# IRVLUTD/GraspTrajOpt

Hardware: AMD Instinct MI355X
Metric: grasp trajectories/sec (higher is better)
Workload: dtype f64

## Files before the change

grasptrajopt_amd/csrc/gto_api.hip:

```cpp
#include <hip/hip_runtime.h>
#include <hipcub/hipcub.hpp>

#include <algorithm>
#include <atomic>
#include <climits>
#include <cmath>
#include <cstdio>
#include <cstdlib>
#include <cstring>
#include <string>
#include <chrono>
#include <memory>
#include <mutex>
#include <thread>
#include <utility>
#include <vector>

#include <sys/prctl.h>

#include "gto_kernels.h"

#define GTO_VERSION GTO_ABI_VERSION
#ifndef GTO_OBS_DEEP_PD
#define GTO_OBS_DEEP_PD 8
// ... 92 lines not shown
  void* p = nullptr;
  size_t cap = 0;
};

struct gto_handle {
  int device = 0;
  hipStream_t stream = nullptr;
  bool own_stream = true;
  std::string err;
  gto_solver_opts opts;
  RobotDev rb;
  RobotDev* d_rb = nullptr;
  double *d_px = nullptr, *d_py = nullptr, *d_pz = nullptr;
  int32_t *d_plink = nullptr, *d_perm = nullptr;
  Chunk* d_chunks = nullptr;
  PbChunk* d_pbchunks = nullptr;
  int pb_C = 0;
  std::vector<SceneDev> scenes;
  SceneDev* d_scenes = nullptr;
  size_t d_scenes_cap = 0;
  DevBuf state, Qcur, Qtry, vis, screw, blocks, goalblk, ssfixed, ndone, qf, livebuf, qfs, wrecbuf, itembuf;
  DevBuf counters;
  unsigned long long last_counters[4] = {0, 0, 0, 0};
  int32_t* h_ndone = nullptr;
  unsigned long long* h_progress = nullptr;
  unsigned long long* d_progress = nullptr;
  unsigned progress_tag = 0;
  Tunables tu;
  int spec_kmax = 1;
  long long* dbg = nullptr;
  std::vector<std::pair<void*, size_t>> spare;
  DevBuf in[8], out[8];
// ... 207 lines not shown
  rb.frame_free_mask = 0u;
  for (int i = 0; i < d->n_frames; ++i)
    if (rb.opt_of_frame[i] < 0) rb.frame_free_mask |= 1u << i;
  for (int i = 0; i < d->n_frames; ++i) {
    const int p = rb.parent[i];
    if (p >= 0 && p != i - 1 && rb.xst_slot[p] < 0) rb.xst_slot[p] = rb.n_xst++;
  }
  {
    for (int i = 0; i < d->n_frames; ++i) {
      const int p = rb.parent[i], l = rb.link_of_frame[i];
      const int src = p < 0 ? 0 : (p == i - 1 ? 1 : 2 + rb.xst_slot[p]);
      const bool moving_link = l >= 0 && (rb.frame_anc[rb.link_frame[l]] != 0u);
      rb.pb_ctl[i] = (src & 7) | (((rb.xst_slot[i] + 1) & 7) << 4) | ((moving_link ? 1 : 0) << 8);
      rb.pb_par[i] = -1;
      if (rb.joint_type[i] != GTO_JOINT_FIXED && rb.opt_of_frame[i] < 0) rb.pb_par[i] = rb.pb_npar, rb.pb_parf[rb.pb_npar++] = i;
    }
    double D = 0.0, maxp = 0.0;
    for (int i = 0; i < d->n_frames; ++i) {
      const double* ox = d->origin_xyz + 3 * i;
      D += std::sqrt(ox[0] * ox[0] + ox[1] * ox[1] + ox[2] * ox[2]);
      if (rb.joint_type[i] == GTO_JOINT_PRISMATIC) {
        const int j = rb.opt_of_frame[i];
        D += j >= 0 ? std::max(std::fabs(rb.lower[j]), std::fabs(rb.upper[j])) : 2.0;
      }
    }
    for (int l = 0; l < d->n_links; ++l) {
      const double* vx = d->visual_xyz + 3 * l;
      maxp = std::max(maxp, std::sqrt(vx[0] * vx[0] + vx[1] * vx[1] + vx[2] * vx[2]));
    }
    double maxr = 0.0;
// ... 256 lines not shown
    while (spec_kmax < GTO_KSPEC && lm_lds_bytes(opts->T, spec_kmax + 1) <= 160 * 1024 - 256) ++spec_kmax;

  int ndev = 0;
  if (hipGetDeviceCount(&ndev) != hipSuccess || ndev == 0)
    return fail(nullptr, GTO_ERR_NO_DEVICE, "no HIP device visible: the GTO solve path has no CPU fallback");
  if (device >= ndev) return fail(nullptr, GTO_ERR_INVALID_ARG, "device index out of range");
  if (device >= 0 && hipSetDevice(device) != hipSuccess) return fail(nullptr, GTO_ERR_HIP, "hipSetDevice failed");

  gto_handle* h = new gto_handle();
  if (device >= 0) h->device = device;
  else (void)hipGetDevice(&h->device);
  h->opts = *opts;
  h->tu = tu;
  std::memcpy(&h->rb, &rb, sizeof rb);
  h->pb_C = t->pb_C;
  h->np = np;
  h->lm_lds = lm_lds;
  h->spec_kmax = spec_kmax;
  if (tu.debug_timing) { (void)hipMalloc((void**)&h->dbg, 256 * sizeof(long long)); (void)hipMemset(h->dbg, 0, 256 * sizeof(long long)); }
  auto up = [&](void** dst, const void* src, size_t bytes) -> bool {
    if (hipMalloc(dst, bytes) != hipSuccess) return false;
    return hipMemcpy(*dst, src, bytes, hipMemcpyHostToDevice) == hipSuccess;
  };
  const size_t P = t->px.size();
  if (hipStreamCreateWithFlags(&h->stream, hipStreamNonBlocking) != hipSuccess) { gto_destroy(h); return fail(nullptr, GTO_ERR_HIP, "hipStreamCreate failed"); }
  const bool ok = up((void**)&h->d_rb, &h->rb, sizeof h->rb) && up((void**)&h->d_px, t->px.data(), P * sizeof(double)) &&
                  up((void**)&h->d_py, t->py.data(), P * sizeof(double)) && up((void**)&h->d_pz, t->pz.data(), P * sizeof(double)) &&
                  up((void**)&h->d_plink, t->plink.data(), P * sizeof(int32_t)) && up((void**)&h->d_perm, t->perm.data(), P * sizeof(int32_t)) &&
                  up((void**)&h->d_chunks, t->chunks.data(), t->chunks.size() * sizeof(Chunk)) &&
                  up((void**)&h->d_pbchunks, t->pbchunks.data(), t->pbchunks.size() * sizeof(PbChunk));
  if (!ok) { gto_destroy(h); return fail(nullptr, GTO_ERR_ALLOC, "device allocation failed in gto_create"); }
  const size_t lds = std::min<size_t>((size_t)lay.total_doubles * sizeof(double), 160 * 1024);
  hipError_t e = hipSuccess;
  for (int v = 0; v < 8 && e == hipSuccess; ++v) e = raise_dynamic_lds((const void*)obstacle_kernel(np, v & 1, v & 2, v & 4), lds);
  if (e == hipSuccess) e = wide ? raise_dynamic_lds((const void*)k_lm_step_wide<16>, lm_lds) : raise_dynamic_lds((const void*)k_lm_step<4, 1>, lm_lds);
  if (e == hipSuccess && !wide) e = raise_dynamic_lds((const void*)k_lm_step<8, GTO_KSPEC>, lm_lds_bytes(opts->T, spec_kmax));
  if (e != hipSuccess) { gto_destroy(h); return fail(nullptr, GTO_ERR_HIP, "hipFuncSetAttribute failed"); }
  *out = h;
  return GTO_OK;
}

void gto_destroy(gto_handle* h) {
  if (!h) return;
  (void)hipSetDevice(h->device);
  if (h->stream) (void)hipStreamSynchronize(h->stream);
// ... 3 lines not shown
      (void)hipFree((void*)s.c_all);
      if (s.r_obs != s.r_all) (void)hipFree((void*)s.r_obs);
      (void)hipFree((void*)s.r_all);
      if (s.d_obs != s.d_all) (void)hipFree((void*)s.d_obs);
      (void)hipFree((void*)s.d_all);
    }
  }
  (void)hipFree(h->d_scenes);
  (void)hipFree(h->d_rb);
  (void)hipFree(h->d_px);
  (void)hipFree(h->d_py);
  (void)hipFree(h->d_pz);
  (void)hipFree(h->d_plink);
  (void)hipFree(h->d_perm);
  (void)hipFree(h->d_chunks);
  (void)hipFree(h->d_pbchunks);
  DevBuf* bufs[] = {&h->zws, &h->counters, &h->state, &h->Qcur, &h->Qtry, &h->vis, &h->screw, &h->blocks, &h->goalblk, &h->ssfixed, &h->ndone, &h->qf, &h->livebuf, &h->qfs, &h->wrecbuf, &h->itembuf};
  if (h->h_ndone) (void)hipHostFree(h->h_ndone);
  if (h->h_progress) (void)hipHostFree(h->h_progress);
  for (DevBuf* b : bufs) (void)hipFree(b->p);
  for (auto& sp_ : h->spare) (void)hipFree(sp_.first);
  for (auto& b : h->in) (void)hipFree(b.p);
  for (auto& b : h->out) (void)hipFree(b.p);
  for (auto& b : h->pin_in) if (b.p) (void)hipHostFree(b.p);
  for (auto& b : h->pin_out) if (b.p) (void)hipHostFree(b.p);
  for (auto e : h->ev) (void)hipEventDestroy(e);
  if (h->stream && h->own_stream) (void)hipStreamDestroy(h->stream);
  for (int l = 0; l < GTO_MAX_LANES; ++l) {
    if (h->lane_stream[l]) (void)hipStreamDestroy(h->lane_stream[l]);
    if (h->lane_event[l]) (void)hipEventDestroy(h->lane_event[l]);
  }
  delete h;
}

int gto_set_opts(gto_handle* h, const gto_solver_opts* o) {
  if (!h || !o) return GTO_ERR_INVALID_ARG;
  std::string why;
  if (!validate_opts(o, why)) return fail(h, GTO_ERR_INVALID_ARG, why);
  if (o->T != h->opts.T) return fail(h, GTO_ERR_INVALID_ARG, "T cannot change after gto_create");
  h->opts = *o;
  return GTO_OK;
}

static int sync_scene_table(gto_handle* h) {
  size_t n = h->scenes.size();
  if (n > h->d_scenes_cap) {
    if (h->d_scenes) HIPCHK(h, hipFree(h->d_scenes));
    h->d_scenes = nullptr;
    size_t cap = std::max<size_t>(16, n * 2);
    HIPCHK(h, hipMalloc((void**)&h->d_scenes, cap * sizeof(SceneDev)));
    h->d_scenes_cap = cap;
  }
  HIPCHK(h, hipMemcpy(h->d_scenes, h->scenes.data(), n * sizeof(SceneDev), hipMemcpyHostToDevice));
  return GTO_OK;
}

static int free_scene(gto_handle* h, SceneDev& s) {
  if (s.valid == 1) {
    if (s.c_obs != s.c_all) HIPCHK(h, hipFree((void*)s.c_obs));
    HIPCHK(h, hipFree((void*)s.c_all));
// ... 611 lines not shown
}

static int enqueue_round(gto_handle* h, const SolveCall& c, LaneCtx& ln, int lane_index, const RoundPlan& p) {
  const int B = c.B, T = c.T;
  SolveParams& lsp = ln.sp;
  lsp.interleave = p.interleave;
  lsp.round = ln.k;
  lsp.parity = ln.k & 1;
  lsp.k_eval = ln.k_prev;
  int rc;
  if ((rc = launch_obstacle(h, ln.st, ln.bp, lsp, B, p.obs))) return rc;
  if (h->profiling && (rc = prof_begin(h, ln.st, p.step == STEP_FEW ? GTO_PROF_STEP_FEW : GTO_PROF_STEP, p.in_flight))) return rc;
  if (p.step == STEP_FEW) {
    lsp.k_acc = p.k_acc, lsp.k_rej = p.k_rej, lsp.spec_streak = p.spec_streak;
    lsp.pb_next = 0, lsp.static_pos = 0;
    hipLaunchKernelGGL((k_lm_step<8, GTO_KSPEC>), dim3(p.span), dim3(512), lm_lds_bytes(T, p.k_next), ln.st, h->d_rb, h->d_pbchunks, ln.bp, lsp, B);
  } else if (p.step == STEP_FULL) {
    lsp.k_acc = lsp.k_rej = 1;
    lsp.pb_next = p.pb_next, lsp.static_pos = p.static_pos;
    hipLaunchKernelGGL((k_lm_step<4, 1>), dim3(p.span), dim3(256), h->lm_lds, ln.st, h->d_rb, h->d_pbchunks, ln.bp, lsp, B);
  } else {
    hipLaunchKernelGGL(k_lm_step_wide<16>, dim3(p.in_flight), dim3(GTO_WIDE_NT), h->lm_lds, ln.st, h->d_rb, ln.bp, lsp, B,
                       (double*)h->zws.p + (size_t)c.lane_zws[lane_index] * (T - 2) * h->np * h->np);
  }
  if (h->profiling && (rc = prof_end(h, ln.st))) return rc;
  ln.span_prev = p.static_pos ? p.span : 0;
  ln.items_ready = p.pb_next;
  ln.k_prev = p.k_next;
  ln.pb_off = p.pb_off;
  ln.ratio_max = p.ratio_max;
  ln.k++;
  return GTO_OK;
}

static void read_progress(unsigned tag, LaneCtx& ln) {
// ... 141 lines not shown
}

static int print_debug_stamps(gto_handle* h, hipStream_t st) {
  HIPCHK(h, hipStreamSynchronize(st));
  long long t[256];
  HIPCHK(h, hipMemcpy(t, h->dbg, sizeof t, hipMemcpyDeviceToHost));
  fprintf(stderr, "[gto dbg] step-kernel phases (cycles) P0+P1 %lld | P2 %lld | diag %lld | dense %lld | back %lld | P4 %lld | P5 %lld | s_dense %lld\n",
          t[1] - t[0], t[2] - t[1], t[3] - t[2], t[4] - t[3], t[5] - t[4], t[6] - t[5], t[7] - t[6], t[9]);
  if (h->np != GTO_NB)
    fprintf(stderr, "[gto dbg] wide step kernel, sweeps (cycles): downward: %lld in %lld dense inversions, sweep %lld | upward: %lld in %lld dense inversions, sweep %lld\n",
            t[56], t[57], t[58], t[59], t[60], t[61]);
  fprintf(stderr, "[gto dbg] solve by wave (cycles from the start of P3): downward sweep: diagonal stretch %lld, its dense blocks %lld | upward sweep %lld | meeting block %lld | back substitution from its start: downward wave dense %lld, diagonal stretch %lld | upward wave %lld\n",
          t[3] - t[2], t[41] - t[2], t[17] - t[2], t[42] - t[4], t[18] - t[42], t[19] - t[42], t[26] - t[42]);
  fprintf(stderr, "[gto dbg] sweeps of the other candidates' waves (2..6) done at (cycles from the start of P3, 0 = no candidate): %lld %lld %lld %lld %lld | barrier passed at %lld\n",
          t[43] ? t[43] - t[2] : 0, t[44] ? t[44] - t[2] : 0, t[45] ? t[45] - t[2] : 0, t[46] ? t[46] - t[2] : 0, t[47] ? t[47] - t[2] : 0, t[4] - t[2]);
  fprintf(stderr, "[gto dbg] broad phase in the step kernel's tail (cycles): entry+tables %lld | barrier %lld | A (local transforms, pass 0) %lld | B (chain) %lld | C (sphere tests) %lld | other passes %lld | outputs %lld\n",
          t[33] - t[6], t[34] - t[33], t[35] - t[34], t[36] - t[35], t[37] - t[36], t[38] - t[37], t[39] - t[38]);
  fprintf(stderr, "[gto dbg] P2 split (cycles): loads+barrier %lld | b-vector+masks %lld | blocks %lld | e,y+barrier %lld\n", t[28] - t[1], t[29] - t[28], t[30] - t[29], t[2] - t[30]);
  fprintf(stderr, "[gto dbg] fk_mfma_tree (cycles): local %lld | rounds %lld %lld %lld %lld | outputs %lld\n", t[21] - t[20], t[22] - t[21], t[23] - t[22], t[24] - t[23], t[25] - t[24], t[27] - t[25]);
  fprintf(stderr, "[gto dbg] longest regular obstacle workgroup of the call: %lld cycles with %lld surviving chunks | goal-term wavefront of instance 0: %lld cycles\n",
          t[40] >> 16, t[40] & 0xffff, t[32] - t[31]);
  if (t[64] || t[65]) {
    long long tot_ = 0;
    for (int i = 64; i < 128; ++i) tot_ += t[i];
    fprintf(stderr, "[gto dbg] regular obstacle workgroups of the call: %lld, none of whose keys got a contribution: %lld | surviving chunks per workgroup (0,1,2,...,63+):", tot_, t[48]);
    for (int i = 64; i < 128; ++i) fprintf(stderr, " %lld", t[i]);
    fprintf(stderr, "\n");
    fprintf(stderr, "[gto dbg] ticks those workgroups ran, summed by surviving chunks (0,1,2,...,63+):");
    for (int i = 192; i < 256; ++i) fprintf(stderr, " %lld", t[i]);
    fprintf(stderr, "\n");
// ... 882 lines not shown
```

grasptrajopt_amd/csrc/gto_device.h:

```cpp
#pragma once
#include <hip/hip_runtime.h>
#include <stdint.h>

#include "../../include/gto_solver.h"

#define GTO_NB 8
#ifndef GTO_BROAD_MARGIN
#define GTO_BROAD_MARGIN 0
#endif
#define GTO_GRAM 28
#define GTO_WAVE 64
#define GTO_FK_STRIDE 64
__host__ __device__ inline int fkx(int f, int e) { return 16 * f + (e ^ (5 * (f & 3))); }

struct RobotDev {
  int32_t n_frames, ndof, n_opt, n_links, n_points, n_chunks, n_gripper_points;
  int32_t frame_ee, frame_gripper;
  int32_t fk_rounds;
  int32_t opt_frame[GTO_MAX_OPT];
  double fk_tab[(GTO_FK_STRIDE + 1) * GTO_MAX_FRAMES + 17 * GTO_MAX_LINKS + 18 * GTO_MAX_OPT];
  double fk_tab_c[(GTO_FK_STRIDE + 1) * GTO_MAX_FRAMES + 17 * GTO_MAX_LINKS + 18 * GTO_MAX_OPT];
  int32_t n_cframes, fk_rounds_c;
  int32_t pb_ctl[GTO_MAX_FRAMES];
  double pb_eps;
  int32_t pb_par[GTO_MAX_FRAMES];
  int32_t pb_parf[GTO_MAX_FRAMES];
  int32_t pb_npar;
  int32_t cf_orig[GTO_MAX_FRAMES];
  int32_t cf_type[GTO_MAX_FRAMES];
  int32_t parent[GTO_MAX_FRAMES];
  int32_t joint_type[GTO_MAX_FRAMES];
  int32_t q_index[GTO_MAX_FRAMES];
  int32_t opt_of_frame[GTO_MAX_FRAMES];
  int32_t link_of_frame[GTO_MAX_FRAMES];
  int32_t xst_slot[GTO_MAX_FRAMES];
  int32_t n_xst;
  uint32_t frame_free_mask;
  int32_t opt_of_dof[GTO_MAX_DOF];
  uint32_t frame_anc[GTO_MAX_FRAMES];
  double origin[GTO_MAX_FRAMES][12];
  double axis_unit[GTO_MAX_FRAMES][3];
  int32_t link_frame[GTO_MAX_LINKS];
// ... 10 lines not shown
struct __attribute__((aligned(32))) VoxelRec {
  double dx, dy, dz;
  float c;
  float pad;
};

struct SceneDev {
  const float* c_all;
  const float* c_obs;
  const VoxelRec* r_all;
  const VoxelRec* r_obs;
  const uint8_t* d_all;
  const uint8_t* d_obs;
  int32_t nx, ny, nz, valid;
  double ox, oy, oz, res, rinv, inv2r;
};

struct Chunk {
  int32_t link, start, count, pad;
  double cx, cy, cz, r;
};

__host__ __device__ inline void aff_mul(const double* a, const double* b, double* c) {
  double r[12];
#pragma unroll
  for (int i = 0; i < 3; ++i) {
#pragma unroll
    for (int j = 0; j < 4; ++j) {
      double s = a[4 * i] * b[j] + a[4 * i + 1] * b[4 + j] + a[4 * i + 2] * b[8 + j];
      if (j == 3) s += a[4 * i + 3];
// ... 47 lines not shown
```

grasptrajopt_amd/csrc/gto_kernels.h:

```cpp
#pragma once
#include <type_traits>

#include "gto_device.h"

template <int NP>
struct Blk {
  static constexpr int JTJ = 0, JTR = NP * NP, SS = NP * NP + NP, STRIDE = NP * NP + NP + 8;
};
#define BLK_JTJ 0
#define BLK_JTR 64
#define BLK_SS 72
#define BLK_STRIDE 80
#define GTO_MAX_ACTIVE 256
#define GTO_MAX_TG 8
#define GTO_MAX_T 96
#ifndef GTO_LIST_CAP
#define GTO_LIST_CAP 64
#endif

#define GTO_KSPEC 4
#define GTO_JOB_SHIFT 28
#define GTO_JOB_SET_SHIFT 24
#define GTO_JOB_MASK 0x00ffffff
#define GTO_JOB_ENTRY(b, set, cand) ((b) | ((set) << GTO_JOB_SET_SHIFT) | ((cand) << GTO_JOB_SHIFT))
// ... 1381 lines not shown
}

#ifndef GTO_PB_BATCH
#define GTO_PB_BATCH 5
#endif
#ifndef GTO_DIAG_BATCH
#define GTO_DIAG_BATCH 4
#endif
#define GTO_PB_PARK 4
struct PbChunk {
  double cx, cy, cz, r;
  int32_t frame, pad;
};
#define GTO_PB_FT 10
#define GTO_PB_FTF 20
__host__ __device__ inline int pb_table_doubles(int F, int Cm, int m, int npar) { return 32 + 4 * Cm + GTO_PB_FT * F + m * npar; }
__host__ __device__ inline size_t lm_lds_bytes(int T, int KL);
__host__ __device__ inline int pb_wp_stride(int F) { return 12 * F + 4; }
struct PbLayout {
  int tab0, pw;
  __host__ __device__ PbLayout(int T, int F, int Cm, int npar) {
    const int m = T - 2, top = (int)(lm_lds_bytes(T, 1) / sizeof(double)), tabs = pb_table_doubles(F, Cm, m, npar);
    if (88 * m + tabs <= top) tab0 = 88 * m, pw = (160 * m) / pb_wp_stride(F);
    else tab0 = 80 * m - tabs, pw = tab0 > 0 ? (2 * tab0) / pb_wp_stride(F) : 0;
    if (pw > m) pw = m;
  }
};
#define GTO_PB_SRC(c) ((c)&7)
#define GTO_PB_PARKTO(c) (((c) >> 4) & 7)
#define GTO_PB_LINK(c) (((c) >> 8) & 1)

__device__ __forceinline__ void pb_sincosf(double x, float& sn, float& cs) {
  const double k = rint(x * 6.36619772367581382433e-01);
  const float r = (float)fma(-k, 6.07710050650619224932e-11, fma(-k, 1.57079632673412561417e+00, x));
  const float z = r * r;
  const float s0 = fmaf(r * z, fmaf(z, fmaf(z, fmaf(z, 2.7557319e-06f, -1.9841270e-04f), 8.3333333e-03f), -1.6666667e-01f), r);
  const float c0 = fmaf(z, fmaf(z, fmaf(z, fmaf(z, 2.4801587e-05f, -1.3888889e-03f), 4.1666667e-02f), -0.5f), 1.f);
  const int q = (int)k & 3;
  sn = (q & 1) ? c0 : s0;
  cs = (q & 1) ? s0 : c0;
  if (q == 1 || q == 2) cs = -cs;
  if (q >= 2) sn = -sn;
}

template <int NT>
__device__ __forceinline__ void prebroad_tail(const RobotDev* __restrict__ rb, const PbChunk* __restrict__ pbc,
                                              const BatchPtrs& bp, const SolveParams& sp, int B, int b, int scene_b, int set_n, int pos_next,
                                              const double* __restrict__ s_qt, double* __restrict__ smem, int tid) {
  typedef float gto_f4 __attribute__((ext_vector_type(4)));
  const int lane = tid & 63;
  const int T = sp.T, m = T - 2, F = rb->n_frames, Cm = sp.pb_C, par = sp.parity;
  const int TG = sp.pb_tg, nG = sp.pb_ng, PW = sp.pb_pw, WS = pb_wp_stride(F);
  float* __restrict__ s_L = reinterpret_cast<float*>(smem);
  double* __restrict__ s_tab = smem + sp.pb_tab0;
  int* __restrict__ s_flag = reinterpret_cast<int*>(s_tab);
  gto_f4* __restrict__ s_ck = reinterpret_cast<gto_f4*>(s_tab + 32);
  int* __restrict__ s_ckf = reinterpret_cast<int*>(s_tab + 32 + 2 * Cm);
  float* __restrict__ s_ft = reinterpret_cast<float*>(s_tab + 32 + 4 * Cm);
  double* __restrict__ s_qp = s_tab + 32 + 4 * Cm + GTO_PB_FT * F;
  const SceneDev sc = bp.scenes[__builtin_amdgcn_readfirstlane(scene_b)];
  const double bx = bp.base_pos[3 * b], by = bp.base_pos[3 * b + 1], bz = bp.base_pos[3 * b + 2];
  const bool dbg_t = bp.dbg && b == 0 && tid == 0;
  const int ctlv = rb->pb_ctl[lane & (GTO_MAX_FRAMES - 1)];
  if (tid < 64) s_flag[tid] = 0;
  for (int c = tid; c < Cm; c += NT) {
    const PbChunk cc = pbc[c];
    gto_f4 v;
    v.x = (float)cc.cx, v.y = (float)cc.cy, v.z = (float)cc.cz;
    v.w = (float)((int)ceil((cc.r + sp.pb_eps) * sc.rinv + 1e-6) + GTO_BROAD_MARGIN);
    s_ck[c] = v;
    s_ckf[c] = cc.frame;
  }
  for (int i = tid; i < F * 16; i += NT) {
    const int f = i >> 4, e = i & 15;
    s_ft[GTO_PB_FTF * f + e] = e < 12 ? (float)rb->origin[f][e] : (e < 15 ? (float)rb->axis_unit[f][e - 12] : __int_as_float(rb->joint_type[f] | ((rb->opt_of_frame[f] + 1) << 4) | ((rb->pb_par[f] + 1) << 9)));
  }
  {
    const double* __restrict__ qf0 = bp.qf + ((size_t)b * T + 2) * F;
    const int npar = sp.pb_npar;
    for (int i = tid; i < m * npar; i += NT) {
      const int sI = i / npar, k = i - sI * npar;
      s_qp[i] = qf0[(size_t)sI * F + rb->pb_parf[k]];
    }
  }
  if (dbg_t) bp.dbg[33] = clock64();
  __syncthreads();
  if (dbg_t) bp.dbg[34] = clock64();
  const int row = tid & 3;
  for (int p0 = 0; p0 < m; p0 += PW) {
    const int pwc = min(PW, m - p0);
    for (int idx = tid; idx < pwc * F; idx += NT) {
      const int w = fast_div(idx, F, sp.pb_mF), f = idx - w * F;
      const gto_f4* __restrict__ ft = reinterpret_cast<const gto_f4*>(s_ft + GTO_PB_FTF * f);
      const gto_f4 o0 = ft[0], o1 = ft[1], o2 = ft[2], ux = ft[3];
      const int tj = __float_as_int(ux.w), jt = tj & 15, j = ((tj >> 4) & 31) - 1, kp = (tj >> 9) - 1;
      gto_f4* __restrict__ Lo = reinterpret_cast<gto_f4*>(s_L + w * WS + 12 * f);
      double qv = 0.0;
      if (jt != GTO_JOINT_FIXED) qv = j >= 0 ? s_qt[(p0 + w) * 8 + j] : s_qp[(p0 + w) * sp.pb_npar + kp];
      float sn = 0.f, cs = 1.f;
      if (jt == GTO_JOINT_REVOLUTE) pb_sincosf(qv, sn, cs);
      const float c1 = 1.f - cs, u0 = ux.x, u1 = ux.y, u2 = ux.z;
      const float R00 = fmaf(c1 * u0, u0, cs), R01 = fmaf(c1 * u0, u1, -sn * u2), R02 = fmaf(c1 * u0, u2, sn * u1);
// ... 65 lines not shown
          if (f + 1 < F) {
            const int fn = min(f + 2, F - 1);
            const gto_f4* __restrict__ Ln = reinterpret_cast<const gto_f4*>(Lw + 12 * fn);
            a0 = Ln[0], b0 = Ln[1], c0 = Ln[2];
            ctl0 = __builtin_amdgcn_readlane(ctlv, fn);
            step(f + 1, ctl1, a1, b1, c1);
          }
        }
      }
    };
    if (rb->n_xst <= 1) walk(std::integral_constant<int, 1>());
    else walk(std::integral_constant<int, GTO_PB_PARK>());
    __syncthreads();
    if (dbg_t && p0 == 0) bp.dbg[36] = clock64();
    const int n_test = pwc * Cm;
    const float box = (float)(bx - sc.ox), boy = (float)(by - sc.oy), boz = (float)(bz - sc.oz), rinv_f = (float)sc.rinv;
    constexpr int PBU = GTO_PB_BATCH;
#pragma unroll 1
    for (int i0 = tid; i0 < n_test; i0 += PBU * NT) {
      int off[PBU], pkd[PBU];
#pragma unroll
      for (int u = 0; u < PBU; ++u) {
        const int idx = i0 + u * NT;
        const bool live = idx < n_test;
        const int ic = live ? idx : 0;
        const int w = fast_div(ic, Cm, sp.pb_mC), c = ic - w * Cm;
        const gto_f4 ck = s_ck[c];
        const int cfr = s_ckf[c];
        const gto_f4* __restrict__ V = reinterpret_cast<const gto_f4*>(s_L + w * WS + 12 * cfr);
        const gto_f4 va = V[0], vb = V[1], vc = V[2];
        const float u0 = (fmaf(va.z, ck.z, fmaf(va.y, ck.y, fmaf(va.x, ck.x, va.w))) + box) * rinv_f;
        const float u1 = (fmaf(vb.z, ck.z, fmaf(vb.y, ck.y, fmaf(vb.x, ck.x, vb.w))) + boy) * rinv_f;
        const float u2 = (fmaf(vc.z, ck.z, fmaf(vc.y, ck.y, fmaf(vc.x, ck.x, vc.w))) + boz) * rinv_f;
        const int k0 = (int)floorf(u0), k1 = (int)floorf(u1), k2 = (int)floorf(u2);
        const int c0 = min(max(k0, 0), sc.nx - 1), c1 = min(max(k1, 0), sc.ny - 1), c2 = min(max(k2, 0), sc.nz - 1);
        off[u] = c2 + sc.nz * (c1 + sc.ny * c0);
        pkd[u] = (int)ck.w | (((p0 + w) / TG) << 8) | ((p0 + w + 2 >= sp.ts ? 1 : 0) << 16) | ((live ? 1 : 0) << 17);
        asm volatile("" : "+v"(off[u]), "+v"(pkd[u]) :: "memory");
      }
      int dd[PBU];
#pragma unroll
      for (int u = 0; u < PBU; ++u)
        dd[u] = ((pkd[u] >> 17) && (pkd[u] & 255) < GTO_DIST_CAP) ? (int)as_global(((pkd[u] >> 16) & 1) ? sc.d_obs : sc.d_all)[off[u]] : 0;
#pragma unroll
      for (int u = 0; u < PBU; ++u)
        if ((pkd[u] >> 17) && dd[u] <= (pkd[u] & 255)) s_flag[(pkd[u] >> 8) & 255] = 1;
    }
    __syncthreads();
    if (dbg_t && p0 == 0) bp.dbg[37] = clock64();
  }
  if (dbg_t) bp.dbg[38] = clock64();
  {
    const double ss_a = bp.ss_fixed[4 * b + 2], ss_o = bp.ss_fixed[4 * b + 3];
    double* __restrict__ wr = bp.wrec + (((size_t)set_n * B + b) * T + 2) * 8;
    for (int i = tid; i < m * 8; i += NT) {
      const int sI = i >> 3;
      if (!s_flag[sI / TG]) wr[i] = (i & 7) == 0 ? 0.0 + (sI + 2 < sp.ts ? ss_a : ss_o) : 0.0;
    }
  }
  if (tid < 64) {
    const bool hit = tid < nG && s_flag[tid] != 0;
    const bool on = tid < nG && (hit || sp.pb_verify);
    const unsigned long long mask = __ballot(on);
    int base = 0;
    if (lane == 0 && mask) base = atomicAdd(bp.nlive + 8 + (1 - par), __popcll(mask));
    base = __shfl(base, 0, 64);
    if (on) bp.items[(size_t)(1 - par) * ((size_t)bp.cap * sp.kcap * (T - 2) + GTO_ITEM_SLACK) + base + __popcll(mask & ((1ull << lane) - 1ull))] =
                make_int2(GTO_JOB_ENTRY(b, set_n, 0), (pos_next << 8) | tid | (hit ? 0 : 0x80));
// ... 110 lines not shown
__device__ __forceinline__ double matvec8(double Z, double zc) {
  double pr = Z * zc;
  pr = dpp_add<0xB1>(pr);
  pr = dpp_add<0x4E>(pr);
  pr = dpp_add<0x141>(pr);
  return pr;
}

__host__ __device__ inline size_t lm_red_doubles(int KL) { return KL == 1 ? 56 : 96; }
__host__ __device__ inline size_t lm_lds_bytes(int T, int KL) {
  const size_t m = (size_t)T - 2;
  const size_t dbl = (size_t)KL * (m * 64 + m * 8) + 3 * m * 8 + 8 * (size_t)T + 16 + lm_red_doubles(KL);
  return dbl * sizeof(double) + ((m + 1) & ~(size_t)1) * sizeof(int);
}
template <int NW, int KC>
__global__ __launch_bounds__(64 * NW, NW == 4 ? 4 : 1) void k_lm_step(const RobotDev* __restrict__ rb, const struct PbChunk* __restrict__ pbc, BatchPtrs bp, SolveParams sp, int B) {
  static_assert(NW >= 2 * KC, "the twisted factorisation of a candidate takes two wavefronts");
  static_assert(KC <= GTO_KSPEC, "candidate copies of the workspace");
  constexpr int NT = 64 * NW;
  const int tid = threadIdx.x, lane = tid & 63, wave = __builtin_amdgcn_readfirstlane(tid >> 6);
  if (blockIdx.x == 0 && threadIdx.x == 0 && bp.progress) {
    const int nd = __hip_atomic_load(bp.n_done, __ATOMIC_RELAXED, __HIP_MEMORY_SCOPE_AGENT);
    __hip_atomic_store(bp.progress, bp.progress_tag | (unsigned long long)(unsigned)nd, __ATOMIC_RELAXED, __HIP_MEMORY_SCOPE_SYSTEM);
    __hip_atomic_store(bp.progress + 1, bp.progress_tag | (unsigned long long)(unsigned)sp.round, __ATOMIC_RELAXED, __HIP_MEMORY_SCOPE_SYSTEM);
    if (bp.items) __hip_atomic_store(bp.progress + 2, bp.progress_tag | ((unsigned long long)min((unsigned)bp.nlive[GTO_NJOBS(sp.parity)], 0xfffu) << 20) | (unsigned long long)min((unsigned)bp.nlive[8 + sp.parity], 0xfffffu),
                                     __ATOMIC_RELAXED, __HIP_MEMORY_SCOPE_SYSTEM);
  }
  const int par = sp.parity, pos_id = blockIdx.x, NS = sp.kcap + 1;
  const int n_live = bp.nlive[GTO_NLIVE(par)], le_ = bp.live[par * bp.cap + min(pos_id, bp.cap - 1)];
  const bool stat = KC == 1 && sp.static_pos != 0;
  if (stat && pos_id == 0 && threadIdx.x == 0) bp.nlive[GTO_NLIVE(1 - par)] = bp.nlive[GTO_NJOBS(1 - par)] = n_live;
// ... 489 lines not shown
      S -= er * ec * cZ[(size_t)(mid + 1) * 64 + lane];
      zc -= ec * cx[(mid + 1) * 8 + c];
    }
    fail |= gj_invert(S);
    const double pr = matvec(S, zc);
    if (c == 0) cx[mid * 8 + r] = pr;
    if (lane == 0) s_red[2 * cj] = __any(fail) ? 1.0 : 0.0;
  }
  __syncthreads();
  if (s_red[0] != 0.0) GTO_FINISH(GTO_STATUS_NUMERICAL);
  if (bp.dbg && b == 0 && tid == 0) bp.dbg[42] = clock64();
  int cflags_new = streak << 16;
#pragma unroll
  for (int j = 1; j < KC; ++j)
    if (j < Kg && s_red[2 * j] != 0.0) cflags_new |= 1 << j;
  if (solver && role == 0) {
    const int nd = s_dense < mid ? s_dense : mid;
    double xr = cx[mid * 8 + r], xc = cx[mid * 8 + c];
    for (int s = mid - 1; s >= nd; --s) {
      const double pr = matvec(cZ[(size_t)s * 64 + lane], s_e[s * 8 + c] * xc);
      xr = cx[s * 8 + r] - pr;
      if (c == 0) cx[s * 8 + r] = xr;
      xc = __shfl(xr, c << 3, 64);
    }
    if (bp.dbg && b == 0 && tid == 0) bp.dbg[18] = clock64();
    if (r == c) {
      int s = nd - 1;
      for (; s >= GTO_DIAG_BATCH - 1; s -= GTO_DIAG_BATCH) {
        double yv[GTO_DIAG_BATCH], zv[GTO_DIAG_BATCH], ev[GTO_DIAG_BATCH];
#pragma unroll
// ... 11 lines not shown
      for (; s >= 0; --s) {
        xr = cx[s * 8 + r] - cZ[(size_t)s * 64 + lane] * (s_e[s * 8 + r] * xr);
        cx[s * 8 + r] = xr;
      }
    }
    if (bp.dbg && b == 0 && tid == 0) bp.dbg[19] = clock64();
  } else if (solver) {
    double xc = cx[mid * 8 + c];
    for (int s = mid + 1; s < m; ++s) {
      const double pr = matvec(cZ[(size_t)s * 64 + lane], s_e[(s - 1) * 8 + c] * xc);
      const double xr = cx[s * 8 + r] - pr;
      if (c == 0) cx[s * 8 + r] = xr;
      xc = __shfl(xr, c << 3, 64);
    }
    if (bp.dbg && b == 0 && tid == 64) bp.dbg[26] = clock64();
  }
  __syncthreads();

  if (bp.dbg && b == 0 && tid == 0) bp.dbg[5] = clock64();
  double* __restrict__ qfn = bp.qfs + ((size_t)(1 - par) * bp.cap * sp.kcap + pos_next) * T * nF;
#pragma unroll
  for (int j = 0; j < KC; ++j)
    if (j < Kg) {
      double* __restrict__ qfj = qfn + (size_t)j * T * nF;
#pragma unroll
      for (int u = 0; u < NFV; ++u)
        if ((fv_keep >> u) & 1u) qfj[tid + NT * u] = fv_[u];
      for (int idx = tid + NT * NFV; idx < T * nF; idx += NT)
        if (idx < 2 * nF || rb->opt_of_frame[idx % nF] < 0) qfj[idx] = bp.qf[(size_t)b * T * nF + idx];
    }
#pragma unroll
  for (int j = 0; j < KC; ++j)
// ... 73 lines not shown
        const double* pr_ = s_red + 48 + 8 * j;
        st->pred[j] = -(((pr_[0] + pr_[1]) + (pr_[2] + pr_[3])) + ((pr_[4] + pr_[5]) + (pr_[6] + pr_[7])));
      }
    st->ncand = Kg;
    st->cflags = cflags_new;
    st->nz0 = nz0, st->nz1 = nz1;
    st->slot = slot;
    st->first = 0;
    st->status = status;
    st->evals = k + 1;
    st->argmin_cur = argmin_cur;
  }
  if constexpr (KC == 1) {
    if (sp.pb_next) {
      __syncthreads();
      prebroad_tail<NT>(rb, pbc, bp, sp, B, b, scene_b, (slot + 1) % NS, pos_next, s_e, smem, tid);
    }
  }
#undef GTO_FINISH
  if (bp.dbg && b == 0 && tid == 0) bp.dbg[7] = clock64();
  if (bp.dbg && b == 0 && tid == 0) {
    bp.dbg[8] = clock64();
    bp.dbg[9] = s_dense;
  }
}

__host__ __device__ inline int ik_lds_doubles(int F, int L, int n) {
  return fk_tab_doubles(F, L, n) + 2 * F + fk_scratch_doubles(F) + L * 12 + GTO_NB * 6 + 24 + 2 * BLK_STRIDE + 4 * L * 8 +
         2 * 64 + 2 * 8 + 8 + 8 + 8 + GTO_MAX_DOF + 16 + L * 8 + L;
}

// ... 1850 lines not shown
```

Baseline: 542,500.

## Precompute broad-phase tables per scene and prefetch them during back substitution

Moves the per-step construction of the broad-phase chunk and frame tables to the host: per-scene float images of the chunk spheres and a float frame table in the robot struct. In the one-candidate step kernel, the otherwise idle waves 2-3 load these tables, the header and the joint values into registers during the back substitution, then stage them in shared memory for the broad-phase tail. This is meant to hide global-load latency and conversion work in the tail. In exchange it adds shared-memory staging, register pressure and extra host work whenever the scene table is synced.

```diff
diff --git a/grasptrajopt_amd/csrc/gto_api.hip b/grasptrajopt_amd/csrc/gto_api.hip
--- a/grasptrajopt_amd/csrc/gto_api.hip
+++ b/grasptrajopt_amd/csrc/gto_api.hip
@@ -130,8 +130,10 @@
   double *d_px = nullptr, *d_py = nullptr, *d_pz = nullptr;
   int32_t *d_plink = nullptr, *d_perm = nullptr;
   Chunk* d_chunks = nullptr;
-  PbChunk* d_pbchunks = nullptr;
+  std::vector<PbChunk> pbchunks;
   int pb_C = 0;
+  float* d_pbimg = nullptr;
+  size_t d_pbimg_cap = 0;
   std::vector<SceneDev> scenes;
   SceneDev* d_scenes = nullptr;
   size_t d_scenes_cap = 0;
@@ -369,6 +371,12 @@
       rb.pb_ctl[i] = (src & 7) | (((rb.xst_slot[i] + 1) & 7) << 4) | ((moving_link ? 1 : 0) << 8);
       rb.pb_par[i] = -1;
       if (rb.joint_type[i] != GTO_JOINT_FIXED && rb.opt_of_frame[i] < 0) rb.pb_par[i] = rb.pb_npar, rb.pb_parf[rb.pb_npar++] = i;
+    }
+    for (int i = 0; i < d->n_frames; ++i) {
+      for (int e = 0; e < 12; ++e) rb.pb_ft[i][e] = (float)rb.origin[i][e];
+      for (int e = 0; e < 3; ++e) rb.pb_ft[i][12 + e] = (float)rb.axis_unit[i][e];
+      const int32_t w = rb.joint_type[i] | ((rb.opt_of_frame[i] + 1) << 4) | ((rb.pb_par[i] + 1) << 9);
+      std::memcpy(&rb.pb_ft[i][15], &w, sizeof w);
     }
     double D = 0.0, maxp = 0.0;
     for (int i = 0; i < d->n_frames; ++i) {
@@ -655,6 +663,7 @@
   h->tu = tu;
   std::memcpy(&h->rb, &rb, sizeof rb);
   h->pb_C = t->pb_C;
+  h->pbchunks = t->pbchunks;
   h->np = np;
   h->lm_lds = lm_lds;
   h->spec_kmax = spec_kmax;
@@ -668,8 +677,7 @@
   const bool ok = up((void**)&h->d_rb, &h->rb, sizeof h->rb) && up((void**)&h->d_px, t->px.data(), P * sizeof(double)) &&
                   up((void**)&h->d_py, t->py.data(), P * sizeof(double)) && up((void**)&h->d_pz, t->pz.data(), P * sizeof(double)) &&
                   up((void**)&h->d_plink, t->plink.data(), P * sizeof(int32_t)) && up((void**)&h->d_perm, t->perm.data(), P * sizeof(int32_t)) &&
-                  up((void**)&h->d_chunks, t->chunks.data(), t->chunks.size() * sizeof(Chunk)) &&
-                  up((void**)&h->d_pbchunks, t->pbchunks.data(), t->pbchunks.size() * sizeof(PbChunk));
+                  up((void**)&h->d_chunks, t->chunks.data(), t->chunks.size() * sizeof(Chunk));
   if (!ok) { gto_destroy(h); return fail(nullptr, GTO_ERR_ALLOC, "device allocation failed in gto_create"); }
   const size_t lds = std::min<size_t>((size_t)lay.total_doubles * sizeof(double), 160 * 1024);
   hipError_t e = hipSuccess;
@@ -703,7 +711,7 @@
   (void)hipFree(h->d_plink);
   (void)hipFree(h->d_perm);
   (void)hipFree(h->d_chunks);
-  (void)hipFree(h->d_pbchunks);
+  (void)hipFree(h->d_pbimg);
   DevBuf* bufs[] = {&h->zws, &h->counters, &h->state, &h->Qcur, &h->Qtry, &h->vis, &h->screw, &h->blocks, &h->goalblk, &h->ssfixed, &h->ndone, &h->qf, &h->livebuf, &h->qfs, &h->wrecbuf, &h->itembuf};
   if (h->h_ndone) (void)hipHostFree(h->h_ndone);
   if (h->h_progress) (void)hipHostFree(h->h_progress);
@@ -731,8 +739,41 @@
   return GTO_OK;
 }
 
+static int sync_pb_images(gto_handle* h) {
+  const int C = h->pb_C;
+  const size_t rows = (size_t)pb_img_rows(C);
+  size_t nv = 0;
+  for (const SceneDev& s : h->scenes) nv += s.valid ? 1 : 0;
+  if (nv * rows * 4 > h->d_pbimg_cap) {
+    if (h->d_pbimg) HIPCHK(h, hipFree(h->d_pbimg));
+    h->d_pbimg = nullptr;
+    const size_t cap = std::max<size_t>(16, nv * 2) * rows * 4;
+    HIPCHK(h, hipMalloc((void**)&h->d_pbimg, cap * sizeof(float)));
+    h->d_pbimg_cap = cap;
+  }
+  std::vector<float> img(nv * rows * 4, 0.f);
+  const double eps = h->rb.pb_eps;
+  size_t k = 0;
+  for (SceneDev& s : h->scenes) {
+    s.pb_img = nullptr;
+    if (!s.valid || rows == 0) continue;
+    float* v = img.data() + k * rows * 4;
+    for (int c = 0; c < C; ++c) {
+      const PbChunk& cc = h->pbchunks[c];
+      v[4 * c] = (float)cc.cx, v[4 * c + 1] = (float)cc.cy, v[4 * c + 2] = (float)cc.cz;
+      v[4 * c + 3] = (float)((int)std::ceil(std::fma(cc.r + eps, s.rinv, 1e-6)) + GTO_BROAD_MARGIN);
+      std::memcpy(v + 4 * C + c, &cc.frame, sizeof(int32_t));
+    }
+    s.pb_img = h->d_pbimg + k * rows * 4;
+    ++k;
+  }
+  if (!img.empty()) HIPCHK(h, hipMemcpy(h->d_pbimg, img.data(), img.size() * sizeof(float), hipMemcpyHostToDevice));
+  return GTO_OK;
+}
+
 static int sync_scene_table(gto_handle* h) {
   size_t n = h->scenes.size();
+  if (int rc = sync_pb_images(h)) return rc;
   if (n > h->d_scenes_cap) {
     if (h->d_scenes) HIPCHK(h, hipFree(h->d_scenes));
     h->d_scenes = nullptr;
@@ -1374,11 +1415,11 @@
   if (p.step == STEP_FEW) {
     lsp.k_acc = p.k_acc, lsp.k_rej = p.k_rej, lsp.spec_streak = p.spec_streak;
     lsp.pb_next = 0, lsp.static_pos = 0;
-    hipLaunchKernelGGL((k_lm_step<8, GTO_KSPEC>), dim3(p.span), dim3(512), lm_lds_bytes(T, p.k_next), ln.st, h->d_rb, h->d_pbchunks, ln.bp, lsp, B);
+    hipLaunchKernelGGL((k_lm_step<8, GTO_KSPEC>), dim3(p.span), dim3(512), lm_lds_bytes(T, p.k_next), ln.st, h->d_rb, ln.bp, lsp, B);
   } else if (p.step == STEP_FULL) {
     lsp.k_acc = lsp.k_rej = 1;
     lsp.pb_next = p.pb_next, lsp.static_pos = p.static_pos;
-    hipLaunchKernelGGL((k_lm_step<4, 1>), dim3(p.span), dim3(256), h->lm_lds, ln.st, h->d_rb, h->d_pbchunks, ln.bp, lsp, B);
+    hipLaunchKernelGGL((k_lm_step<4, 1>), dim3(p.span), dim3(256), h->lm_lds, ln.st, h->d_rb, ln.bp, lsp, B);
   } else {
     hipLaunchKernelGGL(k_lm_step_wide<16>, dim3(p.in_flight), dim3(GTO_WIDE_NT), h->lm_lds, ln.st, h->d_rb, ln.bp, lsp, B,
                        (double*)h->zws.p + (size_t)c.lane_zws[lane_index] * (T - 2) * h->np * h->np);
@@ -1550,6 +1591,8 @@
           t[3] - t[2], t[41] - t[2], t[17] - t[2], t[42] - t[4], t[18] - t[42], t[19] - t[42], t[26] - t[42]);
   fprintf(stderr, "[gto dbg] sweeps of the other candidates' waves (2..6) done at (cycles from the start of P3, 0 = no candidate): %lld %lld %lld %lld %lld | barrier passed at %lld\n",
           t[43] ? t[43] - t[2] : 0, t[44] ? t[44] - t[2] : 0, t[45] ? t[45] - t[2] : 0, t[46] ? t[46] - t[2] : 0, t[47] ? t[47] - t[2] : 0, t[4] - t[2]);
+  fprintf(stderr, "[gto dbg] tail tables fetched by waves 2-3 during the back substitution (cycles from its start): in at %lld %lld | its barrier passed at %lld\n",
+          t[51] ? t[51] - t[42] : 0, t[52] ? t[52] - t[42] : 0, t[5] - t[42]);
   fprintf(stderr, "[gto dbg] broad phase in the step kernel's tail (cycles): entry+tables %lld | barrier %lld | A (local transforms, pass 0) %lld | B (chain) %lld | C (sphere tests) %lld | other passes %lld | outputs %lld\n",
           t[33] - t[6], t[34] - t[33], t[35] - t[34], t[36] - t[35], t[37] - t[36], t[38] - t[37], t[39] - t[38]);
   fprintf(stderr, "[gto dbg] P2 split (cycles): loads+barrier %lld | b-vector+masks %lld | blocks %lld | e,y+barrier %lld\n", t[28] - t[1], t[29] - t[28], t[30] - t[29], t[2] - t[30]);
diff --git a/grasptrajopt_amd/csrc/gto_device.h b/grasptrajopt_amd/csrc/gto_device.h
--- a/grasptrajopt_amd/csrc/gto_device.h
+++ b/grasptrajopt_amd/csrc/gto_device.h
@@ -26,6 +26,7 @@
   int32_t pb_par[GTO_MAX_FRAMES];
   int32_t pb_parf[GTO_MAX_FRAMES];
   int32_t pb_npar;
+  alignas(16) float pb_ft[GTO_MAX_FRAMES][16];
   int32_t cf_orig[GTO_MAX_FRAMES];
   int32_t cf_type[GTO_MAX_FRAMES];
   int32_t parent[GTO_MAX_FRAMES];
@@ -66,6 +67,7 @@
   const uint8_t* d_obs;
   int32_t nx, ny, nz, valid;
   double ox, oy, oz, res, rinv, inv2r;
+  const float* pb_img;
 };
 
 struct Chunk {
diff --git a/grasptrajopt_amd/csrc/gto_kernels.h b/grasptrajopt_amd/csrc/gto_kernels.h
--- a/grasptrajopt_amd/csrc/gto_kernels.h
+++ b/grasptrajopt_amd/csrc/gto_kernels.h
@@ -1419,7 +1419,8 @@
 };
 #define GTO_PB_FT 10
 #define GTO_PB_FTF 20
-__host__ __device__ inline int pb_table_doubles(int F, int Cm, int m, int npar) { return 32 + 4 * Cm + GTO_PB_FT * F + m * npar; }
+__host__ __device__ inline int pb_table_doubles(int F, int Cm, int m, int npar) { return 56 + 4 * Cm + GTO_PB_FT * F + m * npar; }
+__host__ __device__ inline int pb_img_rows(int Cm) { return Cm + (Cm + 3) / 4; }
 __host__ __device__ inline size_t lm_lds_bytes(int T, int KL);
 __host__ __device__ inline int pb_wp_stride(int F) { return 12 * F + 4; }
 struct PbLayout {
@@ -1448,8 +1449,74 @@
   if (q >= 2) sn = -sn;
 }
 
+#ifndef GTO_PB_PRE
+#define GTO_PB_PRE 1
+#endif
+#define GTO_PB_PREQ 2
+typedef float pb_f4 __attribute__((ext_vector_type(4)));
+struct PbPre {
+  pb_f4 v[GTO_PB_PRE];
+  double q[GTO_PB_PREQ];
+  int h;
+};
+__device__ __forceinline__ const pb_f4* pb_row_src(const pb_f4* img, const RobotDev* __restrict__ rb, int u, int nck) {
+  return u < nck ? img + u : reinterpret_cast<const pb_f4*>(&rb->pb_ft[0][0]) + (u - nck);
+}
+__device__ __forceinline__ int pb_row_dst(int u, int nck, int Cm) {
+  return u < nck ? 28 + u : 28 + 2 * Cm + (GTO_PB_FTF / 4) * ((u - nck) >> 2) + ((u - nck) & 3);
+}
+__device__ __forceinline__ int pb_header(const RobotDev* __restrict__ rb, const BatchPtrs& bp, int b, const SceneDev* __restrict__ scp, int i) {
+  if (i >= 16) return rb->pb_ctl[i - 16];
+  const SceneDev sc = *scp;
+  if (i < 4) {
+    const double o = i == 0 ? sc.ox : (i == 1 ? sc.oy : sc.oz);
+    return __float_as_int(i < 3 ? (float)(bp.base_pos[3 * b + i] - o) : (float)sc.rinv);
+  }
+  if (i < 8) return i == 4 ? sc.nx : (i == 5 ? sc.ny : (i == 6 ? sc.nz : 0));
+  const unsigned long long w = i < 10 ? (unsigned long long)sc.d_obs : (i < 12 ? (unsigned long long)sc.d_all :
+                               (unsigned long long)__double_as_longlong(bp.ss_fixed[4 * b + 2 + ((i - 12) >> 1)]));
+  return (int)(unsigned)(w >> (32 * (i & 1)));
+}
+#define GTO_PB_STAGE (24 + 2 * 128 * GTO_PB_PRE + 128 * GTO_PB_PREQ)
+__host__ __device__ inline bool pb_pre_on(int T, int tab0) { return 64 * (T - 2) >= GTO_PB_STAGE && tab0 >= GTO_PB_STAGE; }
+__device__ __forceinline__ void pb_stage(const PbPre& pre, double* __restrict__ smem, int t2) {
+  if (t2 < 48) reinterpret_cast<int*>(smem)[t2] = pre.h;
+#pragma unroll
+  for (int k = 0; k < GTO_PB_PRE; ++k) reinterpret_cast<pb_f4*>(smem + 24)[t2 + 128 * k] = pre.v[k];
+#pragma unroll
+  for (int k = 0; k < GTO_PB_PREQ; ++k) (smem + 24 + 256 * GTO_PB_PRE)[t2 + 128 * k] = pre.q[k];
+}
+__device__ __forceinline__ void pb_prefetch(const RobotDev* __restrict__ rb, const BatchPtrs& bp, const SolveParams& sp, int b,
+                                            int scene_b, int t2, PbPre& pre) {
+  const int F = rb->n_frames, Cm = sp.pb_C, nck = pb_img_rows(Cm), nrow = nck + 4 * F, npar = sp.pb_npar, nq = (sp.T - 2) * npar;
+  const SceneDev* __restrict__ scp = bp.scenes + __builtin_amdgcn_readfirstlane(scene_b);
+  const pb_f4* __restrict__ img = reinterpret_cast<const pb_f4*>(scp->pb_img);
+#pragma unroll
+  for (int k = 0; k < GTO_PB_PRE; ++k) {
+    const int u = t2 + 128 * k;
+    pre.v[k] = u < nrow ? *pb_row_src(img, rb, u, nck) : pb_f4{0.f, 0.f, 0.f, 0.f};
+  }
+  const double* __restrict__ qf0 = bp.qf + ((size_t)b * sp.T + 2) * F;
+#pragma unroll
+  for (int k = 0; k < GTO_PB_PREQ; ++k) {
+    const int i = t2 + 128 * k;
+    double v = 0.0;
+    if (i < nq) {
+      const int sI = i / npar, kk = i - sI * npar;
+      v = qf0[(size_t)sI * F + rb->pb_parf[kk]];
+    }
+    pre.q[k] = v;
+  }
+  pre.h = t2 < 48 ? pb_header(rb, bp, b, scp, t2) : 0;
+#pragma unroll
+  for (int k = 0; k < GTO_PB_PRE; ++k) asm volatile("" : "+v"(pre.v[k]));
+#pragma unroll
+  for (int k = 0; k < GTO_PB_PREQ; ++k) asm volatile("" : "+v"(pre.q[k]));
+  asm volatile("" : "+v"(pre.h));
+}
+
 template <int NT>
-__device__ __forceinline__ void prebroad_tail(const RobotDev* __restrict__ rb, const PbChunk* __restrict__ pbc,
+__device__ __forceinline__ void prebroad_tail(const RobotDev* __restrict__ rb,
                                               const BatchPtrs& bp, const SolveParams& sp, int B, int b, int scene_b, int set_n, int pos_next,
                                               const double* __restrict__ s_qt, double* __restrict__ smem, int tid) {
   typedef float gto_f4 __attribute__((ext_vector_type(4)));
@@ -1459,31 +1526,34 @@
   float* __restrict__ s_L = reinterpret_cast<float*>(smem);
   double* __restrict__ s_tab = smem + sp.pb_tab0;
   int* __restrict__ s_flag = reinterpret_cast<int*>(s_tab);
-  gto_f4* __restrict__ s_ck = reinterpret_cast<gto_f4*>(s_tab + 32);
-  int* __restrict__ s_ckf = reinterpret_cast<int*>(s_tab + 32 + 2 * Cm);
-  float* __restrict__ s_ft = reinterpret_cast<float*>(s_tab + 32 + 4 * Cm);
-  double* __restrict__ s_qp = s_tab + 32 + 4 * Cm + GTO_PB_FT * F;
-  const SceneDev sc = bp.scenes[__builtin_amdgcn_readfirstlane(scene_b)];
-  const double bx = bp.base_pos[3 * b], by = bp.base_pos[3 * b + 1], bz = bp.base_pos[3 * b + 2];
+  int* __restrict__ s_hdr = reinterpret_cast<int*>(s_tab + 32);
+  gto_f4* __restrict__ s_ck = reinterpret_cast<gto_f4*>(s_tab + 56);
+  int* __restrict__ s_ckf = reinterpret_cast<int*>(s_tab + 56 + 2 * Cm);
+  float* __restrict__ s_ft = reinterpret_cast<float*>(s_tab + 56 + 4 * Cm);
+  double* __restrict__ s_qp = s_tab + 56 + 4 * Cm + GTO_PB_FT * F;
   const bool dbg_t = bp.dbg && b == 0 && tid == 0;
-  const int ctlv = rb->pb_ctl[lane & (GTO_MAX_FRAMES - 1)];
-  if (tid < 64) s_flag[tid] = 0;
-  for (int c = tid; c < Cm; c += NT) {
-    const PbChunk cc = pbc[c];
-    gto_f4 v;
-    v.x = (float)cc.cx, v.y = (float)cc.cy, v.z = (float)cc.cz;
-    v.w = (float)((int)ceil((cc.r + sp.pb_eps) * sc.rinv + 1e-6) + GTO_BROAD_MARGIN);
-    s_ck[c] = v;
-    s_ckf[c] = cc.frame;
-  }
-  for (int i = tid; i < F * 16; i += NT) {
-    const int f = i >> 4, e = i & 15;
-    s_ft[GTO_PB_FTF * f + e] = e < 12 ? (float)rb->origin[f][e] : (e < 15 ? (float)rb->axis_unit[f][e - 12] : __int_as_float(rb->joint_type[f] | ((rb->opt_of_frame[f] + 1) << 4) | ((rb->pb_par[f] + 1) << 9)));
-  }
+  static_assert(NT == 256, "waves 2-3 of the one-candidate step kernel carry the tables");
   {
+    const int nck = pb_img_rows(Cm), nrow = nck + 4 * F, npar = sp.pb_npar, nq = m * npar;
+    const bool pre_on = pb_pre_on(T, sp.pb_tab0);
+    const int nr0 = pre_on ? min(nrow, 128 * GTO_PB_PRE) : 0, nq0 = pre_on ? min(nq, 128 * GTO_PB_PREQ) : 0;
+    gto_f4* __restrict__ s_tab4 = reinterpret_cast<gto_f4*>(s_tab);
+    if (tid < 64) s_flag[tid] = 0;
+    if (pre_on) {
+      const gto_f4* __restrict__ g_v = reinterpret_cast<const gto_f4*>(smem + 24);
+      const double* __restrict__ g_q = smem + 24 + 256 * GTO_PB_PRE;
+      for (int u = tid; u < nr0; u += NT) s_tab4[pb_row_dst(u, nck, Cm)] = g_v[u];
+      for (int i = tid; i < nq0; i += NT) s_qp[i] = g_q[i];
+      if (tid < 24) s_tab[32 + tid] = smem[tid];
+    }
+    const SceneDev* __restrict__ scp = bp.scenes + __builtin_amdgcn_readfirstlane(scene_b);
+    if (!pre_on && tid < 48) s_hdr[tid] = pb_header(rb, bp, b, scp, tid);
+    if (nrow > nr0) {
+      const gto_f4* __restrict__ img = reinterpret_cast<const gto_f4*>(scp->pb_img);
+      for (int u = nr0 + tid; u < nrow; u += NT) s_tab4[pb_row_dst(u, nck, Cm)] = *pb_row_src(img, rb, u, nck);
+    }
     const double* __restrict__ qf0 = bp.qf + ((size_t)b * T + 2) * F;
-    const int npar = sp.pb_npar;
-    for (int i = tid; i < m * npar; i += NT) {
+    for (int i = nq0 + tid; i < nq; i += NT) {
       const int sI = i / npar, k = i - sI * npar;
       s_qp[i] = qf0[(size_t)sI * F + rb->pb_parf[k]];
     }
@@ -1491,6 +1561,15 @@
   if (dbg_t) bp.dbg[33] = clock64();
   __syncthreads();
   if (dbg_t) bp.dbg[34] = clock64();
+  const int ctlv = s_hdr[16 + (lane & (GTO_MAX_FRAMES - 1))];
+  const float box = __int_as_float(s_hdr[0]), boy = __int_as_float(s_hdr[1]), boz = __int_as_float(s_hdr[2]), rinv_f = __int_as_float(s_hdr[3]);
+  const int snx = __builtin_amdgcn_readfirstlane(s_hdr[4]), sny = __builtin_amdgcn_readfirstlane(s_hdr[5]), snz = __builtin_amdgcn_readfirstlane(s_hdr[6]);
+  auto hdr_ptr = [&](int i) {
+    return reinterpret_cast<const uint8_t*>(((unsigned long long)(unsigned)__builtin_amdgcn_readfirstlane(s_hdr[i + 1]) << 32) |
+                                            (unsigned)__builtin_amdgcn_readfirstlane(s_hdr[i]));
+  };
+  const uint8_t* __restrict__ d_obs = hdr_ptr(8);
+  const uint8_t* __restrict__ d_all = hdr_ptr(10);
   const int row = tid & 3;
   for (int p0 = 0; p0 < m; p0 += PW) {
     const int pwc = min(PW, m - p0);
@@ -1586,7 +1665,6 @@
     __syncthreads();
     if (dbg_t && p0 == 0) bp.dbg[36] = clock64();
     const int n_test = pwc * Cm;
-    const float box = (float)(bx - sc.ox), boy = (float)(by - sc.oy), boz = (float)(bz - sc.oz), rinv_f = (float)sc.rinv;
     constexpr int PBU = GTO_PB_BATCH;
 #pragma unroll 1
     for (int i0 = tid; i0 < n_test; i0 += PBU * NT) {
@@ -1605,15 +1683,15 @@
         const float u1 = (fmaf(vb.z, ck.z, fmaf(vb.y, ck.y, fmaf(vb.x, ck.x, vb.w))) + boy) * rinv_f;
         const float u2 = (fmaf(vc.z, ck.z, fmaf(vc.y, ck.y, fmaf(vc.x, ck.x, vc.w))) + boz) * rinv_f;
         const int k0 = (int)floorf(u0), k1 = (int)floorf(u1), k2 = (int)floorf(u2);
-        const int c0 = min(max(k0, 0), sc.nx - 1), c1 = min(max(k1, 0), sc.ny - 1), c2 = min(max(k2, 0), sc.nz - 1);
-        off[u] = c2 + sc.nz * (c1 + sc.ny * c0);
+        const int c0 = min(max(k0, 0), snx - 1), c1 = min(max(k1, 0), sny - 1), c2 = min(max(k2, 0), snz - 1);
+        off[u] = c2 + snz * (c1 + sny * c0);
         pkd[u] = (int)ck.w | (((p0 + w) / TG) << 8) | ((p0 + w + 2 >= sp.ts ? 1 : 0) << 16) | ((live ? 1 : 0) << 17);
         asm volatile("" : "+v"(off[u]), "+v"(pkd[u]) :: "memory");
       }
       int dd[PBU];
 #pragma unroll
       for (int u = 0; u < PBU; ++u)
-        dd[u] = ((pkd[u] >> 17) && (pkd[u] & 255) < GTO_DIST_CAP) ? (int)as_global(((pkd[u] >> 16) & 1) ? sc.d_obs : sc.d_all)[off[u]] : 0;
+        dd[u] = ((pkd[u] >> 17) && (pkd[u] & 255) < GTO_DIST_CAP) ? (int)as_global(((pkd[u] >> 16) & 1) ? d_obs : d_all)[off[u]] : 0;
 #pragma unroll
       for (int u = 0; u < PBU; ++u)
         if ((pkd[u] >> 17) && dd[u] <= (pkd[u] & 255)) s_flag[(pkd[u] >> 8) & 255] = 1;
@@ -1623,7 +1701,7 @@
   }
   if (dbg_t) bp.dbg[38] = clock64();
   {
-    const double ss_a = bp.ss_fixed[4 * b + 2], ss_o = bp.ss_fixed[4 * b + 3];
+    const double ss_a = s_tab[38], ss_o = s_tab[39];
     double* __restrict__ wr = bp.wrec + (((size_t)set_n * B + b) * T + 2) * 8;
     for (int i = tid; i < m * 8; i += NT) {
       const int sI = i >> 3;
@@ -1764,7 +1842,7 @@
   return dbl * sizeof(double) + ((m + 1) & ~(size_t)1) * sizeof(int);
 }
 template <int NW, int KC>
-__global__ __launch_bounds__(64 * NW, NW == 4 ? 4 : 1) void k_lm_step(const RobotDev* __restrict__ rb, const struct PbChunk* __restrict__ pbc, BatchPtrs bp, SolveParams sp, int B) {
+__global__ __launch_bounds__(64 * NW, NW == 4 ? 4 : 1) void k_lm_step(const RobotDev* __restrict__ rb, BatchPtrs bp, SolveParams sp, int B) {
   static_assert(NW >= 2 * KC, "the twisted factorisation of a candidate takes two wavefronts");
   static_assert(KC <= GTO_KSPEC, "candidate copies of the workspace");
   constexpr int NT = 64 * NW;
@@ -2284,6 +2362,8 @@
 #pragma unroll
   for (int j = 1; j < KC; ++j)
     if (j < Kg && s_red[2 * j] != 0.0) cflags_new |= 1 << j;
+  const bool pb_pre = KC == 1 && sp.pb_next && pb_pre_on(T, sp.pb_tab0);
+  PbPre pre;
   if (solver && role == 0) {
     const int nd = s_dense < mid ? s_dense : mid;
     double xr = cx[mid * 8 + r], xc = cx[mid * 8 + c];
@@ -2325,8 +2405,16 @@
       xc = __shfl(xr, c << 3, 64);
     }
     if (bp.dbg && b == 0 && tid == 64) bp.dbg[26] = clock64();
+  } else if constexpr (KC == 1) {
+    if (pb_pre) {
+      pb_prefetch(rb, bp, sp, b, scene_b, tid - NT / 2, pre);
+      if (bp.dbg && b == 0 && lane == 0) bp.dbg[49 + wave] = clock64();
+    }
   }
   __syncthreads();
+  if constexpr (KC == 1) {
+    if (pb_pre && wave >= 2) pb_stage(pre, smem, tid - NT / 2);
+  }
 
   if (bp.dbg && b == 0 && tid == 0) bp.dbg[5] = clock64();
   double* __restrict__ qfn = bp.qfs + ((size_t)(1 - par) * bp.cap * sp.kcap + pos_next) * T * nF;
@@ -2430,7 +2518,7 @@
   if constexpr (KC == 1) {
     if (sp.pb_next) {
       __syncthreads();
-      prebroad_tail<NT>(rb, pbc, bp, sp, B, b, scene_b, (slot + 1) % NS, pos_next, s_e, smem, tid);
+      prebroad_tail<NT>(rb, bp, sp, B, b, scene_b, (slot + 1) % NS, pos_next, s_e, smem, tid);
     }
   }
 #undef GTO_FINISH
```

After: 551,100 (median of 6 runs). +1.6%, better.
